# DCGM/pero-pretraining

Hardware: AMD Instinct MI355X
Metric: text-line images/sec (masked-ViT step) (higher is better)
Workload: dtype bf16; 1 GPU; masked pretraining step incl. prepare_batch, 12-layer d=512 h=4 ff=2048 ViT, V=4096, 40x2048 u8 lines (BASELINE.json configs[1]); uint8 images resident in HBM, the PCIe-inclusive rate is `with_h2d`; lines_per_gpu=2048, global_batch=2048, seq_len=256, parallelism=dp1, optimizer=fused Adam (f32 master weights), weight_gradients_on_side_stream=False, head_rows=all, head_backward=masked

## Files before the change

pero_pretraining_amd/csrc/attention.hip:

```cpp
#include "common.hpp"

#define AT_HALF_BYTES 16384
#ifndef AT_NO_PRIO
#define AT_PRIO(n_) __builtin_amdgcn_s_setprio(n_)
#else
#define AT_PRIO(n_)
#endif
#define AT_SUB_BYTES 8192
#ifndef AT_COLSUM_MFMA
#define AT_COLSUM_MFMA 1
#endif
#ifndef AT_ABL
#define AT_ABL 0
#endif
#define AT_DKV2_LDS (4 * AT_SUB_BYTES + 128 * 128 * 2 + 512)
#define AT_TILE_BYTES (128 * 128 * 2)

template <bool VIMG>
__device__ __forceinline__ void attn_glds_tile(const bf16raw* g, long long ld, unsigned char* lds, int wave, int lane) {
#pragma unroll
  for (int i = 0; i < 8; i++) {
    const int p = wave + 4 * i;
    const int row = 4 * p + (lane >> 4), slot = lane & 15;
    const int chunk = VIMG ? ((((slot >> 2) ^ (row & 3)) << 2) | (slot & 3)) : (slot ^ (row & 15));
// ... 1418 lines not shown
  bf8v qf[8];
  const unsigned qoff = (unsigned)((long long)q * ld * 2 + 16 * h5);
  auto load_q = [&](int head) {
    const bf16raw* qb_ = lbase + head * 128;
    at_static_for<0, 8>([&](auto kc) __attribute__((always_inline)) { constexpr int ks = decltype(kc)::value; lh_gload16<32 * ks>(qf[ks], qb_, qoff); });
  };
  load_q(head0);
  const unsigned kbase = at_lds_addr(kimg), vbase = at_lds_addr(vimg);
  const unsigned ka0 = (unsigned)(r * 256 + ((h5 ^ (r & 15)) << 4));
  unsigned va0;
  {
    const int i = lane & 15, g1 = (lane >> 4) & 1;
    const int key = 4 * h5 + (i >> 2);
    va0 = (unsigned)(key * 256 + ((key & 3) << 6) + g1 * 32 + (i & 3) * 8);
  }
  f16v o[4];
#pragma unroll
  for (int t = 0; t < 4; t++) o[t] = (f16v){0};
  float m = -INFINITY, l = 0.f;

  for (int u = 0; u < units; u++) {
    const int head = head0 + u / nkt, kt = u % nkt;
    if (u > 0) asm volatile("s_waitcnt vmcnt(8)" ::: "memory");
    else asm volatile("s_waitcnt vmcnt(0)" ::: "memory");
    asm volatile("" : "+v"(qf[0]), "+v"(qf[1]), "+v"(qf[2]), "+v"(qf[3]), "+v"(qf[4]), "+v"(qf[5]), "+v"(qf[6]), "+v"(qf[7]) :: "memory");
    lh_barrier();
    bf8v fr[FW_POOL];
    f16v s[4];
    auto issue_k = [&](auto jc) __attribute__((always_inline)) {
      constexpr int j = decltype(jc)::value;
      constexpr int t = j >> 3, ks = j & 7;
      at_rd128x<t * 8192, 32 * ks>(fr[j % FW_POOL], ka0, kbase);
    };
    at_static_for<0, 6>(issue_k);
    AT_PRIO(1);
    at_static_for<0, 32>([&](auto jc) __attribute__((always_inline)) {
      constexpr int j = decltype(jc)::value;
      constexpr int t = j >> 3, ks = j & 7;
      if constexpr (j + 6 < 32) issue_k(std::integral_constant<int, j + 6>{});
      constexpr int after = (31 - j) < 6 ? (31 - j) : 6;
      at_wait_lgkm<after>(fr[j % FW_POOL]);
      if constexpr (ks == 0) s[t] = __builtin_amdgcn_mfma_f32_32x32x16_bf16(fr[j % FW_POOL], qf[0], (f16v){0}, 0, 0, 0);
      else s[t] = __builtin_amdgcn_mfma_f32_32x32x16_bf16(fr[j % FW_POOL], qf[ks], s[t], 0, 0, 0);
    });
    AT_PRIO(0);
    asm volatile("s_waitcnt vmcnt(0)" ::: "memory");
    lh_barrier();
    if (u + 1 < units) {
      const int nhd = head0 + (u + 1) / nkt, nkt_i = (u + 1) % nkt;
      attn_glds_tile<false>(lbase + nhd * 128 + d + (long long)nkt_i * 128 * ld, ld, kimg, wave, lane);
    }
    auto issue_v = [&](auto mc) __attribute__((always_inline)) {
      constexpr int mm = decltype(mc)::value;
      constexpr int t = mm >> 3, sub = (mm >> 2) & 1, dt = mm & 3;
      at_rdtrx<t * 8192 + sub * 4096, t * 8192 + sub * 4096 + 2048, 64 * dt>(fr[mm % FW_POOL], va0, va0, vbase);
    };
    at_static_for<0, 7>(issue_v);

    float mx = s[0][0];
#pragma unroll
    for (int t = 0; t < 4; t++)
#pragma unroll
      for (int e = 0; e < 16; e++) mx = fmaxf(mx, s[t][e]);
    {
      const auto sw = __builtin_amdgcn_permlane32_swap(__float_as_uint(mx), __float_as_uint(mx), false, false);
      mx = fmaxf(__uint_as_float(sw[0]), __uint_as_float(sw[1]));
    }
    const float mn = fmaxf(m, mx);
    const float alpha = __builtin_amdgcn_exp2f((m - mn) * c);
    const float mc = mn * c;
    float ps = 0.f;
#pragma unroll
    for (int t = 0; t < 4; t++)
#pragma unroll
      for (int e = 0; e < 16; e++) {
        const float p = __builtin_amdgcn_exp2f(fmaf(s[t][e], c, -mc));
        s[t][e] = p;
        ps += p;
      }
    {
      const auto sw = __builtin_amdgcn_permlane32_swap(__float_as_uint(ps), __float_as_uint(ps), false, false);
      ps = __uint_as_float(sw[0]) + __uint_as_float(sw[1]);
    }
    l = l * alpha + ps;
    m = mn;
    if (kt != 0) {
#pragma unroll
      for (int t = 0; t < 4; t++)
#pragma unroll
        for (int e = 0; e < 16; e++) o[t][e] *= alpha;
    }

    AT_PRIO(1);
    at_static_for<0, 32>([&](auto mc_) __attribute__((always_inline)) {
      constexpr int mm = decltype(mc_)::value;
      constexpr int t = mm >> 3, sub = (mm >> 2) & 1, dt = mm & 3;
      if constexpr (mm + 7 < 32) issue_v(std::integral_constant<int, mm + 7>{});
      constexpr int after = 2 * ((31 - mm) < 7 ? (31 - mm) : 7);
      at_wait_lgkm<after>(fr[mm % FW_POOL]);
      const bf8v pf = pack8(s[t], sub);
      o[dt] = __builtin_amdgcn_mfma_f32_32x32x16_bf16(fr[mm % FW_POOL], pf, o[dt], 0, 0, 0);
    });
    AT_PRIO(0);
    if (kt == nkt - 1) {
      lh_barrier();
      const float inv = 1.0f / l;
      int qrow_l = wave * 32 + r, tid_l = tid;
      asm volatile("" : "+v"(qrow_l), "+v"(tid_l));
#pragma unroll
      for (int dt = 0; dt < 4; dt++)
#pragma unroll
        for (int g4 = 0; g4 < 4; g4++) {
          const at_u2v w = {pack2bf(o[dt][4 * g4 + 0] * inv, o[dt][4 * g4 + 1] * inv), pack2bf(o[dt][4 * g4 + 2] * inv, o[dt][4 * g4 + 3] * inv)};
          const int g = dt * 8 + 2 * g4 + h5;
          lh_ds_write8(vbase + qrow_l * 256 + ((g ^ (qrow_l & 31)) << 3), w);
        }
      lh_gstore4(m * c + __builtin_amdgcn_logf(l), lse2 + ((long long)line * nh + head) * S, (unsigned)q * 4u);
      lh_wait_lgkm_plain<0>();
      lh_barrier();
      {
        const int ch = tid_l & 15;
        at_u4v v[8];
#pragma unroll
        for (int i = 0; i < 8; i++) {
          const int row = (tid_l >> 4) + 16 * i;
          lh_ds_read16(v[i], vbase + row * 256 + ((ch ^ ((row & 31) >> 1)) << 4));
        }
        asm volatile("s_waitcnt lgkmcnt(0)" : "+v"(v[0]), "+v"(v[1]), "+v"(v[2]), "+v"(v[3]), "+v"(v[4]), "+v"(v[5]), "+v"(v[6]), "+v"(v[7]) :: "memory");
#pragma unroll
        for (int i = 0; i < 8; i++) {
          const int row = (tid_l >> 4) + 16 * i;
          at_u4v x = v[i];
          if (row & 1) x = (at_u4v){v[i][2], v[i][3], v[i][0], v[i][1]};
          lh_gstore16<0>(x, out + ((long long)line * S + qb * 128) * d + head * 128, (unsigned)(row * (int)d * 2 + ch * 16));
        }
      }
      if (u + 1 < units) {
#pragma unroll
        for (int t = 0; t < 4; t++) o[t] = (f16v){0};
        m = -INFINITY;
        l = 0.f;
        load_q(head + 1);
      }
    }
    if (u + 1 < units) {
      lh_barrier();
      const int nhd = head0 + (u + 1) / nkt, nkt_i = (u + 1) % nkt;
      attn_glds_tile<true>(lbase + nhd * 128 + 2 * d + (long long)nkt_i * 128 * ld, ld, vimg, wave, lane);
    }
  }
}


int g_attn_bwd_pair = 1;
int g_attn_order = 32;
int g_attn_lh = 0;
int g_attn_pipe = 1;
extern "C" int pero_attention_bwd(const void* qkv, const void* out, const void* dout, const float* lse, float* dvec, void* dqkv,
                                  float* dbias, float* work, int64_t N, int64_t S, int64_t num_heads, int64_t head_dim, int dtype,
                                  void* stream) {
  PERO_REQUIRE(qkv && dout && lse && dvec && dqkv, "pero_attention_bwd: null pointer");
  PERO_REQUIRE(dtype == PERO_BF16 && head_dim == 128 && S % 128 == 0 && S > 0 && N > 0 && num_heads > 0,
               "pero_attention_bwd: fused kernel needs bf16, head_dim 128, S %% 128 == 0");
  PERO_REQUIRE(aligned16(qkv) && (!out || aligned16(out)) && aligned16(dout) && aligned16(dqkv), "pero_attention_bwd: 16-byte alignment");
  PERO_REQUIRE(!dbias || work, "pero_attention_bwd: dbias needs the partial-sum workspace");
  PERO_LDS_ATTR(attn_bwd_dq_k<false>, 2 * AT_TILE_BYTES);
  PERO_LDS_ATTR(attn_bwd_dq_k<true>, 2 * AT_TILE_BYTES);
  PERO_LDS_ATTR(attn_bwd_dkv2_k<false>, AT_DKV2_LDS);
  PERO_LDS_ATTR(attn_bwd_dkv2_k<true>, AT_DKV2_LDS);
  PERO_LDS_ATTR(attn_bwd_pair_k<false>, AT_DKV2_LDS > 2 * AT_TILE_BYTES ? AT_DKV2_LDS : 2 * AT_TILE_BYTES);
  PERO_LDS_ATTR(attn_bwd_pair_k<true>, AT_DKV2_LDS > 2 * AT_TILE_BYTES ? AT_DKV2_LDS : 2 * AT_TILE_BYTES);
  const float scale = (float)(1.0 / sqrt((double)head_dim));
  const float c = (float)(1.4426950408889634 / sqrt((double)head_dim));
  hipStream_t st = (hipStream_t)stream;
  dim3 grid((unsigned)(N * num_heads * (S / 128))), block(256);
  if (!out && g_attn_bwd_pair && g_attn_lh && S == 256 && dbias && N * num_heads < (1LL << 20) && num_heads <= 1024) {
#ifdef LH_STAMP
#define LH_LAUNCH_LDS (LH_LDS_BYTES + 512)
#else
#define LH_LAUNCH_LDS LH_LDS_BYTES
#endif
    PERO_LDS_ATTR(attn_bwd_lh_k, LH_LAUNCH_LDS);
    const long long units = N * num_heads;
    const int cus = pero_num_cus();
    hipLaunchKernelGGL(attn_bwd_lh_k, dim3((unsigned)(units < cus ? units : cus)), dim3(512), LH_LAUNCH_LDS, st, (const bf16raw*)qkv, (const bf16raw*)dout, lse,
                       (const float*)dvec, (bf16raw*)dqkv, work, (int)units, (int)num_heads, c, scale);
    hipLaunchKernelGGL(attn_bias_reduce_k, dim3((unsigned)num_heads, 3, N >= 4096 ? 128 : N >= 1024 ? 64 : 16), dim3(128), 0, st, work, dbias, (int)N, (int)num_heads, 1);
    PERO_CHECK_LAUNCH("pero_attention_bwd");
    return PERO_OK;
  }
  if (!out && g_attn_bwd_pair) {
    const size_t lds = AT_DKV2_LDS > 2 * AT_TILE_BYTES ? AT_DKV2_LDS : 2 * AT_TILE_BYTES;
    if (g_attn_pipe)
      hipLaunchKernelGGL(attn_bwd_pair_k<true>, dim3(2 * grid.x), block, lds, st, (const bf16raw*)qkv, (const bf16raw*)dout, lse, dvec, (bf16raw*)dqkv,
                         dbias ? work : nullptr, (int)S, (int)num_heads, c, scale, g_attn_order);
    else
      hipLaunchKernelGGL(attn_bwd_pair_k<false>, dim3(2 * grid.x), block, lds, st, (const bf16raw*)qkv, (const bf16raw*)dout, lse, dvec, (bf16raw*)dqkv,
                         dbias ? work : nullptr, (int)S, (int)num_heads, c, scale, g_attn_order);
  } else {
  if (g_attn_pipe)
    hipLaunchKernelGGL(attn_bwd_dq_k<true>, grid, block, 2 * AT_TILE_BYTES, st, (const bf16raw*)qkv, (const bf16raw*)out, (const bf16raw*)dout, lse,
                       dvec, (bf16raw*)dqkv, dbias ? work : nullptr, (int)S, (int)num_heads, c, scale);
  else
    hipLaunchKernelGGL(attn_bwd_dq_k<false>, grid, block, 2 * AT_TILE_BYTES, st, (const bf16raw*)qkv, (const bf16raw*)out, (const bf16raw*)dout, lse,
                       dvec, (bf16raw*)dqkv, dbias ? work : nullptr, (int)S, (int)num_heads, c, scale);
  if (g_attn_pipe)
    hipLaunchKernelGGL(attn_bwd_dkv2_k<true>, grid, block, AT_DKV2_LDS, st, (const bf16raw*)qkv, (const bf16raw*)dout, lse, dvec,
                       (bf16raw*)dqkv, dbias ? work : nullptr, (int)S, (int)num_heads, c, scale);
  else
    hipLaunchKernelGGL(attn_bwd_dkv2_k<false>, grid, block, AT_DKV2_LDS, st, (const bf16raw*)qkv, (const bf16raw*)dout, lse, dvec,
                       (bf16raw*)dqkv, dbias ? work : nullptr, (int)S, (int)num_heads, c, scale);
  }
  if (dbias)
    hipLaunchKernelGGL(attn_bias_reduce_k, dim3((unsigned)num_heads, 3, (N * (S / 128) >= 4096) ? 128 : (N * (S / 128) >= 1024) ? 64 : 16), dim3(128), 0, st, work, dbias, (int)N, (int)num_heads, (int)(S / 128));
  PERO_CHECK_LAUNCH("pero_attention_bwd");
  return PERO_OK;
}
```

pero_pretraining_amd/csrc/gemm.hip:

```cpp
#include "common.hpp"

#include "gemm_common.hpp"
#include <string.h>

#define T_BM 128
#define T_BN 128
#define T_BK 64
#define T_OPBYTES (128 * 64 * 2)
#define T_BUFBYTES (2 * T_OPBYTES)
#define T_EPI_PITCH 528
#define T_LDS_BYTES (128 * T_EPI_PITCH)

__device__ __forceinline__ bf8v frag_rowmajor(const unsigned char* base, int row, int ks, int lane) {
  const int r = row + (lane & 15);
  const int chunk = ks * 4 + (lane >> 4);
  return *(const bf8v*)(base + r * 128 + ((chunk ^ (r & 7)) << 4));
}
__device__ __forceinline__ bf8v frag_kmajor(const unsigned char* base, int col, int ks, int lane) {
  const int i = lane & 15;
  const int krow = ks * 32 + 8 * (lane >> 4) + (i >> 2);
  const unsigned char* a = base + krow * 256 + ((((col >> 4) ^ fk(krow))) << 5) + 8 * (i & 3);
  s4v lo = __builtin_amdgcn_ds_read_tr16_b64_v4i16(LDS_PTR(s4v, a));
  s4v hi = __builtin_amdgcn_ds_read_tr16_b64_v4i16(LDS_PTR(s4v, a + 4 * 256));
  typedef short s8v __attribute__((ext_vector_type(8)));
// ... 135 lines not shown
          case 5: STORE_PREV_BATCH(5); break;
          case 6: STORE_PREV_BATCH(6); break;
          case 7: STORE_PREV_BATCH(7); break;
          default: break;
        }
      }
      const unsigned char* sa = smem + buf * T_BUFBYTES;
      const unsigned char* sb = sa + T_OPBYTES;
      unsigned char* da = smem + (buf ^ 1) * T_BUFBYTES;
      if (t + 1 < it.nk) {
        stage_glds<TA>(it.A, p.lda, it.tm0, it.kbeg + (long long)(t + 1) * T_BK, da, tid);
        stage_glds<TB>(it.B, p.ldb, it.tn0, it.kbeg + (long long)(t + 1) * T_BK, da + T_OPBYTES, tid);
      } else if (have_next && !atomic) {
        stage_glds<TA>(nx.A, p.lda, nx.tm0, nx.kbeg, da, tid);
        stage_glds<TB>(nx.B, p.ldb, nx.tn0, nx.kbeg, da + T_OPBYTES, tid);
      }
#pragma unroll
      for (int ks = 0; ks < 2; ks++) {
        bf8v fa[4], fb[4];
#pragma unroll
        for (int i = 0; i < 4; i++) {
          fa[i] = TA ? frag_kmajor(sa, wm * 64 + i * 16, ks, lane) : frag_rowmajor(sa, wm * 64 + i * 16, ks, lane);
          fb[i] = TB ? frag_kmajor(sb, wn * 64 + i * 16, ks, lane) : frag_rowmajor(sb, wn * 64 + i * 16, ks, lane);
        }
#pragma unroll
        for (int i = 0; i < 4; i++)
#pragma unroll
          for (int j = 0; j < 4; j++)
            acc[i][j] = __builtin_amdgcn_mfma_f32_16x16x32_bf16(fb[j], fa[i], acc[i][j], 0, 0, 0);
      }
      buf ^= 1;
    }
    if (have_prev && it.nk < 8) {
      if (it.nk <= 0) STORE_PREV_BATCH(0);
      if (it.nk <= 1) STORE_PREV_BATCH(1);
      if (it.nk <= 2) STORE_PREV_BATCH(2);
      if (it.nk <= 3) STORE_PREV_BATCH(3);
      if (it.nk <= 4) STORE_PREV_BATCH(4);
      if (it.nk <= 5) STORE_PREV_BATCH(5);
      if (it.nk <= 6) STORE_PREV_BATCH(6);
      if (it.nk <= 7) STORE_PREV_BATCH(7);
    }
    have_prev = false;

    if (atomic) {
      lds_barrier();
#pragma unroll
      for (int i = 0; i < 4; i++)
#pragma unroll
        for (int j = 0; j < 4; j++)
          *(f4v*)(smem + (lm + i * 16) * T_EPI_PITCH + (ln + j * 16) * 4) = acc[i][j];
      lds_barrier();
      float* C = (float*)p.C + it.coff;
#pragma unroll 4
      for (int i = 0; i < 32; i++) {
        const int row = wave + 4 * i;
#pragma unroll
        for (int j = 0; j < 2; j++) {
          const int col = lane + 64 * j;
          const float v = *(const float*)(smem + row * T_EPI_PITCH + col * 4) * p.alpha;
          atomicAdd(C + (it.tm0 + row) * p.ldc + it.tn0 + col, v);
        }
      }
      if (have_next) {
        lds_barrier();
        stage_glds<TA>(nx.A, p.lda, nx.tm0, nx.kbeg, smem, tid);
        stage_glds<TB>(nx.B, p.ldb, nx.tn0, nx.kbeg, smem + T_OPBYTES, tid);
        buf = 0;
      }
    } else {
#pragma unroll
      for (int i = 0; i < 4; i++)
#pragma unroll
        for (int j = 0; j < 4; j++) prev[i][j] = acc[i][j];
      pm = it.tm0 + lm; pn = it.tn0 + ln; pcoff = it.coff;
      have_prev = true;
    }
    if (!have_next) break;
    w = wnext;
    it = nx;
  }
  if (have_prev) {
#pragma unroll
    for (int b = 0; b < 8; b++) { STORE_PREV_BATCH(b); }
  }
#undef STORE_PREV
#undef STORE_PREV_BATCH
}

template <typename TI, typename TO>
__global__ __launch_bounds__(256) void gemm_generic(GemmP p) {
  __shared__ float As[64][17];
  __shared__ float Bs[64][17];
  const int tid = threadIdx.x, lane = tid & 63, wave = tid >> 6;
  const int wm = wave >> 1, wn = wave & 1;
  const long long tm0 = (long long)blockIdx.x * 64, tn0 = (long long)blockIdx.y * 64;
  const int b = blockIdx.z;
  const long long bo = b / p.binner, bi = b % p.binner;
  const TI* A = (const TI*)p.A + bo * p.sAo + bi * p.sAi;
  const TI* B = (const TI*)p.B + bo * p.sBo + bi * p.sBi;
  const long long coff = bo * p.sCo + bi * p.sCi;
  const bool ta = p.flags & PERO_GEMM_TRANS_A, tb = p.flags & PERO_GEMM_TRANS_B;
  const long long sam = ta ? 1 : p.lda, sak = ta ? p.lda : 1;
  const long long sbn = tb ? 1 : p.ldb, sbk = tb ? p.ldb : 1;

  f16v acc = {0};
  for (long long k0 = 0; k0 < p.K; k0 += 16) {
#pragma unroll
    for (int i = 0; i < 4; i++) {
      const int idx = tid + 256 * i;
      int m, k;
      if (ta) { m = idx & 63; k = idx >> 6; } else { m = idx >> 4; k = idx & 15; }
      float v = 0.f;
      if (tm0 + m < p.M && k0 + k < p.K) v = Elem<TI>::ld(A + (tm0 + m) * sam + (k0 + k) * sak);
      As[m][k] = v;
      int n, k2;
      if (tb) { n = idx & 63; k2 = idx >> 6; } else { n = idx >> 4; k2 = idx & 15; }
      float w = 0.f;
      if (tn0 + n < p.N && k0 + k2 < p.K) w = Elem<TI>::ld(B + (tn0 + n) * sbn + (k0 + k2) * sbk);
      Bs[n][k2] = w;
    }
    __syncthreads();
#pragma unroll
    for (int k = 0; k < 16; k += 2) {
      const float a = As[wm * 32 + (lane & 31)][k + (lane >> 5)];
      const float bb = Bs[wn * 32 + (lane & 31)][k + (lane >> 5)];
      acc = __builtin_amdgcn_mfma_f32_32x32x2f32(a, bb, acc, 0, 0, 0);
    }
    __syncthreads();
  }
  const long long n = tn0 + wn * 32 + (lane & 31);
  if (n >= p.N) return;
  const float bias = p.bias ? p.bias[n] : 0.f;
#pragma unroll
  for (int r = 0; r < 16; r++) {
    const long long m = tm0 + wm * 32 + (r & 3) + 8 * (r >> 2) + 4 * (lane >> 5);
    if (m >= p.M) continue;
    float v = acc[r] * p.alpha + bias;
    if (p.resid) v += Elem<TI>::ld((const TI*)p.resid + coff + m * p.ldr + n);
    if (p.flags & PERO_GEMM_RELU) v = fmaxf(v, 0.f);
    if (p.gate && !(Elem<TI>::ld((const TI*)p.gate + coff + m * p.ldg + n) > 0.f)) v = 0.f;
    TO* c = (TO*)p.C + coff + m * p.ldc + n;
    if (sizeof(TO) == 4 && (p.flags & PERO_GEMM_ATOMIC)) atomicAdd((float*)c, v);
    else if (sizeof(TO) == 4 && (p.flags & PERO_GEMM_ACCUM)) *(float*)c += v;
    else Elem<TO>::st(c, v);
  }
}

extern int g_gemm_e_var;
extern int g_attn_bwd_pair;
extern int g_attn_pipe;
extern int g_attn_order;
extern int g_attn_lh;
extern int g_gemm_splitk_ws;
extern int g_gemm_splitk_table;
extern int g_gemm_nw;
extern int g_gemm_d128;
extern int g_gemm_e_walk;
static int g_gemm_policy = 0;
static int g_gemm_e256_min = 192;
static int g_gemm_e_splitk_min = 4;
static int g_splitk_items = 512;
static int g_splitk_nearest = 0;
int g_pero_splitk_xcd = 1;
extern "C" int pero_set_option(const char* name, int value) {
  if (name && !strcmp(name, "gemm_policy")) { g_gemm_policy = value; return PERO_OK; }
  if (name && !strcmp(name, "gemm_e_var")) { g_gemm_e_var = value; return PERO_OK; }
  if (name && !strcmp(name, "attn_bwd_pair")) { g_attn_bwd_pair = value; return PERO_OK; }
  if (name && !strcmp(name, "attn_pipe")) { g_attn_pipe = value; return PERO_OK; }
  if (name && !strcmp(name, "attn_order")) { g_attn_order = value; return PERO_OK; }
  if (name && !strcmp(name, "attn_lh")) { g_attn_lh = value; return PERO_OK; }
  if (name && !strcmp(name, "splitk_workspace")) { g_gemm_splitk_ws = value; return PERO_OK; }
  if (name && !strcmp(name, "splitk_table")) { g_gemm_splitk_table = value; return PERO_OK; }
  if (name && !strcmp(name, "gemm_nw")) { g_gemm_nw = value; return PERO_OK; }
  if (name && !strcmp(name, "gemm_d128")) { g_gemm_d128 = value; return PERO_OK; }
  if (name && !strcmp(name, "gemm_e_walk")) { g_gemm_e_walk = value; return PERO_OK; }
  if (name && !strcmp(name, "gemm_e256_min")) { g_gemm_e256_min = value; return PERO_OK; }
  if (name && !strcmp(name, "gemm_e_splitk_min")) { g_gemm_e_splitk_min = value; return PERO_OK; }
  if (name && !strcmp(name, "splitk_xcd")) { g_pero_splitk_xcd = value; return PERO_OK; }
  if (name && !strcmp(name, "splitk_nearest")) { g_splitk_nearest = value; return PERO_OK; }
  if (name && !strcmp(name, "splitk_items")) { g_splitk_items = value > 0 ? value : 512; return PERO_OK; }
  pero_set_error("pero_set_option: unknown option %s", name ? name : "(null)");
  return PERO_E_INVALID;
}

static int gemm_dispatch(const void* A, const void* B, void* C, const float* bias, const void* residual, const void* gate,
                         int64_t M, int64_t N, int64_t K, int64_t lda, int64_t ldb, int64_t ldc, int64_t ldr, int64_t ldg,
                         int64_t batch, int64_t batch_inner,
                         int64_t sAo, int64_t sAi, int64_t sBo, int64_t sBi, int64_t sCo, int64_t sCi,
                         float alpha, int flags, int k_split, int in_dtype, int out_dtype, void* workspace, int64_t workspace_bytes,
                         void* stream, bool* colsum_fused);

static bool splitk_takes_e256(int64_t M, int64_t N, int64_t K, int flags) {
  const bool can256 = M % 256 == 0 && N % 256 == 0 && !(flags & PERO_GEMM_TILE128) && g_gemm_policy != 1;
  const long long t256 = can256 ? (M / 256) * (N / 256) : 0;
  return can256 && K % 64 == 0 && K >= 128 &&
         (g_gemm_policy == 20 || (g_gemm_policy == 0 && ((flags & PERO_GEMM_TILE256) || (g_gemm_e256_min > 0 && K >= 32768 && t256 >= g_gemm_e_splitk_min))));
}
extern "C" int pero_gemm_resid_layernorm(const void* A, const void* W, const float* bias, const void* R, const float* gamma, const float* beta,
                                         void* Y, void* T, float* mean, float* rstd, int64_t M, int64_t N, int64_t K, int64_t lda, int64_t ldw,
                                         int64_t ldy, int64_t ldr, int64_t ldt, float eps, void* stream) {
  PERO_REQUIRE(A && W && R && gamma && beta && T && mean && rstd, "pero_gemm_resid_layernorm: null pointer");
  PERO_REQUIRE(N == 512 && M > 0 && M % 128 == 0 && K % 64 == 0 && K >= 192 && lda % 8 == 0 && ldw % 8 == 0 && (!Y || ldy % 8 == 0) && ldr % 8 == 0 &&
               ldt % 8 == 0 && aligned16(A) && aligned16(W) && aligned16(R) && (!Y || aligned16(Y)) && aligned16(T) && aligned16(gamma) && aligned16(beta) &&
               (!bias || aligned16(bias)),
               "pero_gemm_resid_layernorm: bf16, N = 512, M %% 128 == 0, K %% 64 == 0, K >= 192, 16-byte aligned rows");
  GemmP p;
  p.A = A; p.B = W; p.C = Y; p.bias = bias; p.resid = R; p.gate = nullptr;
  p.M = M; p.N = N; p.K = K; p.lda = lda; p.ldb = ldw; p.ldc = Y ? ldy : 512; p.ldr = ldr; p.ldg = 0;
  p.sAo = p.sAi = p.sBo = p.sBi = p.sCo = p.sCi = 0;
  p.binner = 1; p.alpha = 1.0f; p.flags = 0; p.kchunk = K;
  PERO_REQUIRE(pero_launch_gemm_n512_ln(p, T, ldt, mean, rstd, gamma, beta, eps, (hipStream_t)stream), "pero_gemm_resid_layernorm: shape not taken");
  PERO_CHECK_LAUNCH("pero_gemm_resid_layernorm");
  return PERO_OK;
}
extern "C" int pero_gemm_resid_layernorm_bwd(const void* A, const void* Wt, const void* R, const void* T, const float* rstd, const float* gamma,
                                             const float* beta, void* DX, float* dgamma, float* dbeta, float* dxsum, float* work, int64_t M, int64_t N,
                                             int64_t K, int64_t lda, int64_t ldw, int64_t ldr, int64_t ldt, int64_t lddx, void* stream) {
  PERO_REQUIRE(A && Wt && R && T && rstd && gamma && beta && DX && dgamma && dbeta && work, "pero_gemm_resid_layernorm_bwd: null pointer");
  PERO_REQUIRE(N == 512 && M > 0 && M % 128 == 0 && K % 64 == 0 && K >= 192 && lda % 8 == 0 && ldw % 8 == 0 && ldr % 8 == 0 && ldt % 8 == 0 &&
               lddx % 8 == 0 && aligned16(A) && aligned16(Wt) && aligned16(R) && aligned16(T) && aligned16(DX) && aligned16(gamma) && aligned16(beta),
               "pero_gemm_resid_layernorm_bwd: bf16, N = 512, M %% 128 == 0, K %% 64 == 0, K >= 192, 16-byte aligned rows");
  GemmP p;
  p.A = A; p.B = Wt; p.C = DX; p.bias = nullptr; p.resid = R; p.gate = nullptr;
  p.M = M; p.N = N; p.K = K; p.lda = lda; p.ldb = ldw; p.ldc = lddx; p.ldr = ldr; p.ldg = 0;
  p.sAo = p.sAi = p.sBo = p.sBi = p.sCo = p.sCi = 0;
  p.binner = 1; p.alpha = 1.0f; p.flags = 0; p.kchunk = K;
  int grid = 0;
  PERO_REQUIRE(pero_launch_gemm_n512_lnb(p, T, ldt, rstd, gamma, beta, work, &grid, (hipStream_t)stream), "pero_gemm_resid_layernorm_bwd: shape not taken");
  pero_ln_bwd_reduce_launch(work, dgamma, dbeta, dxsum, grid, 512, (hipStream_t)stream);
  PERO_CHECK_LAUNCH("pero_gemm_resid_layernorm_bwd");
  return PERO_OK;
}
extern "C" int64_t pero_gemm_workspace_bytes(int64_t M, int64_t N, int64_t K, int64_t batch, int flags, int k_split, int in_dtype,
                                             int out_dtype) {
  if (!(flags & PERO_GEMM_ATOMIC) || batch != 1 || in_dtype != PERO_BF16 || out_dtype != PERO_F32 || (flags & PERO_GEMM_FORCE_GENERIC) || M <= 0 ||
      N <= 0 || K <= 0 || !splitk_takes_e256(M, N, K, flags))
    return 0;
  return pero_gemm_e256_splitk_ws_bytes(M, N, K, k_split);
}

extern "C" int pero_gemm(const void* A, const void* B, void* C, const float* bias, const void* residual, const void* gate,
                         int64_t M, int64_t N, int64_t K, int64_t lda, int64_t ldb, int64_t ldc, int64_t ldr, int64_t ldg,
                         int64_t batch, int64_t batch_inner,
                         int64_t sAo, int64_t sAi, int64_t sBo, int64_t sBi, int64_t sCo, int64_t sCi,
                         float alpha, int flags, int k_split, int in_dtype, int out_dtype, void* workspace, int64_t workspace_bytes,
                         void* stream) {
  bool fused = false;
  PERO_REQUIRE(workspace_bytes >= 0 && (workspace || workspace_bytes == 0), "pero_gemm: workspace_bytes without a workspace");
  if (flags & PERO_GEMM_COLSUM)
    PERO_REQUIRE(bias && batch == 1 && !(flags & (PERO_GEMM_ATOMIC | PERO_GEMM_ACCUM | PERO_GEMM_ROWDOT)),
                 "pero_gemm: PERO_GEMM_COLSUM needs the output pointer in `bias`, one problem, a stored result");
  if (flags & PERO_GEMM_ROWDOT)
    PERO_REQUIRE(bias && gate && batch == 1 && out_dtype == PERO_BF16 && N % 128 == 0 && !(flags & (PERO_GEMM_ATOMIC | PERO_GEMM_ACCUM)),
                 "pero_gemm: PERO_GEMM_ROWDOT needs the output pointer in `bias`, the second matrix in `gate`, bf16 C, N %% 128 == 0");
  const int rc = gemm_dispatch(A, B, C, bias, residual, gate, M, N, K, lda, ldb, ldc, ldr, ldg, batch, batch_inner, sAo, sAi, sBo, sBi,
                               sCo, sCi, alpha, flags, k_split, in_dtype, out_dtype, workspace, workspace_bytes, stream, &fused);
  if (rc != PERO_OK || !(flags & (PERO_GEMM_COLSUM | PERO_GEMM_ROWDOT)) || fused) return rc;
  if (flags & PERO_GEMM_ROWDOT) return pero_rowdot_blocks(C, gate, (float*)bias, M, N, ldc, ldg, stream);
  return pero_colsum(C, (float*)bias, M, N, ldc, out_dtype, stream);
}

static int gemm_dispatch(const void* A, const void* B, void* C, const float* bias, const void* residual, const void* gate,
                         int64_t M, int64_t N, int64_t K, int64_t lda, int64_t ldb, int64_t ldc, int64_t ldr, int64_t ldg,
                         int64_t batch, int64_t batch_inner,
                         int64_t sAo, int64_t sAi, int64_t sBo, int64_t sBi, int64_t sCo, int64_t sCi,
                         float alpha, int flags, int k_split, int in_dtype, int out_dtype, void* workspace, int64_t workspace_bytes,
                         void* stream, bool* colsum_fused) {
  PERO_REQUIRE(A && B && C, "pero_gemm: null operand");
  PERO_REQUIRE(M > 0 && N > 0 && K > 0 && batch > 0 && batch_inner > 0, "pero_gemm: bad sizes M=%lld N=%lld K=%lld batch=%lld",
               (long long)M, (long long)N, (long long)K, (long long)batch);
  PERO_REQUIRE((in_dtype == PERO_F32 || in_dtype == PERO_BF16) && (out_dtype == PERO_F32 || out_dtype == PERO_BF16), "pero_gemm: bad dtype");
  PERO_REQUIRE(!((flags & (PERO_GEMM_ATOMIC | PERO_GEMM_ACCUM)) && out_dtype != PERO_F32), "pero_gemm: ATOMIC/ACCUM need f32 C");
  PERO_REQUIRE(k_split >= 0 && (k_split == 1 || (flags & PERO_GEMM_ATOMIC)), "pero_gemm: k_split != 1 needs PERO_GEMM_ATOMIC");
  PERO_REQUIRE(batch < 65536, "pero_gemm: batch too large");
  const bool ta = flags & PERO_GEMM_TRANS_A, tb = flags & PERO_GEMM_TRANS_B;
  GemmP p;
  p.A = A; p.B = B; p.C = C; p.bias = bias; p.resid = residual; p.gate = gate;
  p.M = M; p.N = N; p.K = K; p.lda = lda; p.ldb = ldb; p.ldc = ldc; p.ldr = ldr; p.ldg = ldg;
  p.sAo = sAo; p.sAi = sAi; p.sBo = sBo; p.sBi = sBi; p.sCo = sCo; p.sCi = sCi;
  p.binner = (int)batch_inner; p.alpha = alpha; p.flags = flags; p.kchunk = K;
  hipStream_t st = (hipStream_t)stream;
  const bool want_cs = flags & (PERO_GEMM_COLSUM | PERO_GEMM_ROWDOT);
  const bool want_rd = flags & PERO_GEMM_ROWDOT;
  const int cs_bits = flags & (PERO_GEMM_COLSUM | PERO_GEMM_ROWDOT);
  GemmP pc = p;
  if (want_cs) { flags &= ~(PERO_GEMM_COLSUM | PERO_GEMM_ROWDOT); p.flags = flags; p.bias = nullptr; if (want_rd) p.gate = nullptr; }

  const int esz_o = out_dtype == PERO_F32 ? 4 : 2;
  bool fast = in_dtype == PERO_BF16 && !(flags & 32) && M % T_BM == 0 && N % T_BN == 0 && K % T_BK == 0 &&
              lda % 8 == 0 && ldb % 8 == 0 && (ldc * esz_o) % 16 == 0 && aligned16(A) && aligned16(B) && aligned16(C) &&
              (sAo % 8 == 0) && (sAi % 8 == 0) && (sBo % 8 == 0) && (sBi % 8 == 0) && ((sCo * esz_o) % 16 == 0) &&
              ((sCi * esz_o) % 16 == 0) && (!residual || (ldr % 8 == 0 && aligned16(residual))) &&
              (!gate || (flags & PERO_GEMM_RELU_BITS) || (ldg % 8 == 0 && aligned16(gate))) && (!(residual || gate) || out_dtype == PERO_BF16 || true);
  if (fast && g_gemm_policy == 1) { flags |= PERO_GEMM_TILE128; p.flags = flags; pc.flags = flags | cs_bits; }
  const bool force128 = flags & PERO_GEMM_TILE128, force256 = flags & PERO_GEMM_TILE256;
  PERO_REQUIRE(!(flags & PERO_GEMM_MASK_TILED) || ((flags & PERO_GEMM_RELU_BITS) && N % 256 == 0), "pero_gemm: PERO_GEMM_MASK_TILED needs PERO_GEMM_RELU_BITS and N %% 256 == 0");
  if (flags & PERO_GEMM_RELU_BITS) {
    PERO_REQUIRE(fast && gate && batch == 1 && out_dtype == PERO_BF16 && !ta && !(flags & PERO_GEMM_ATOMIC) && !force128 && M % 256 == 0 &&
                 N % 128 == 0 && K % 32 == 0 && !(flags & PERO_GEMM_ROWDOT) && (g_gemm_policy == 0 || g_gemm_policy == 7 || g_gemm_policy == 20),
                 "pero_gemm: PERO_GEMM_RELU_BITS needs a bf16 product for the 256-row tile kernels (M %% 256, N %% 128, K %% 32, batch 1)");
  }
  if (fast) {
    const bool atomic = flags & PERO_GEMM_ATOMIC;
    const bool can256 = M % 256 == 0 && N % 256 == 0 && !force128;
    const long long t256 = can256 ? (M / 256) * (N / 256) * batch : 0;
    const long long t128 = (M / T_BM) * (N / T_BN) * batch;
    const int k_split_req = k_split;
    const bool auto_or = g_gemm_policy == 0;
    if (atomic && out_dtype == PERO_F32 && batch == 1 && splitk_takes_e256(M, N, K, flags) &&
        pero_launch_gemm_e256(p, batch, k_split_req, ta, tb, true, st, -1, workspace, workspace_bytes)) {
      PERO_CHECK_LAUNCH("pero_gemm(e256 split-K)");
      return PERO_OK;
    }
    if (!atomic && g_gemm_nw && !want_cs && out_dtype == PERO_BF16 && pero_launch_gemm_n512(p, batch, ta, tb, false, st)) {
      PERO_CHECK_LAUNCH("pero_gemm(n512)");
      return PERO_OK;
    }
    if (!atomic && g_gemm_d128 && out_dtype == PERO_BF16 && !want_rd && K <= g_gemm_d128 * 64LL && (auto_or || g_gemm_policy == 20) &&
        pero_launch_gemm_d128(pc, batch, ta, tb, false, st)) {
      *colsum_fused = want_cs;
      PERO_CHECK_LAUNCH("pero_gemm(d128)");
      return PERO_OK;
    }
// ... 69 lines not shown
```

Measured before the change: 14190 lines/s.

## Add one-pass fused attention backward kernel for S=256, enabled by default

Adds a new attention-backward kernel that computes dQ, dK, dV and the bias-gradient partials in a single pass per (line, head). K stays resident in LDS, while Q/dO stages and the LSE/dvec statistics are double-buffered. dQ is accumulated through a dS strip in LDS and handled by alternating wave groups. It replaces the two-block pair kernel for S=256, which is meant to remove the repeated loads of Q/K/V/dO and the separate dQ pass. In exchange it uses about 145KB of LDS and 512-thread blocks, which may limit occupancy.

```diff
diff --git a/pero_pretraining_amd/csrc/attention.hip b/pero_pretraining_amd/csrc/attention.hip
--- a/pero_pretraining_amd/csrc/attention.hip
+++ b/pero_pretraining_amd/csrc/attention.hip
@@ -1594,10 +1594,254 @@
 }
 
 
+#define OP_K 0
+#define OP_ST 65536
+#define OP_STAT (OP_ST + 2 * 16384)
+#define OP_STRIP (OP_STAT + 512)
+#define OP_DQS (OP_STRIP + 2 * 16384)
+#define OP_LDS_BYTES (OP_DQS + 2 * 8192)
+#ifndef OP_RDEPTH
+#define OP_RDEPTH 4
+#endif
+#ifndef OP_TDEPTH
+#define OP_TDEPTH 4
+#endif
+
+__device__ __forceinline__ void op_glds(const bf16raw* g, long long ld, unsigned char* lds, int npieces, int wave, int lane) {
+  asm volatile("" : "+v"(lane));
+  for (int p = wave; p < npieces; p += 8) {
+    const int row = 4 * p + (lane >> 4), slot = lane & 15;
+    const int chunk = slot ^ img_f(row);
+    __builtin_amdgcn_global_load_lds((const __attribute__((address_space(1))) void*)((const unsigned char*)g + (unsigned)(row * (int)ld * 2 + chunk * 16)),
+                                     (__attribute__((address_space(3))) void*)(lds + p * 1024), 16, 0, 0);
+  }
+}
+
+__global__ __launch_bounds__(512, 2) void attn_bwd_1p_k(const bf16raw* qkv, const bf16raw* dout, const float* lse2, const float* dvec,
+                                                        bf16raw* dqkv, float* dbias, int nh, float c, float scale) {
+  extern __shared__ __attribute__((aligned(16))) unsigned char smem[];
+  constexpr int S = 256, NST = 8;
+  const int tid = threadIdx.x, lane = tid & 63, h5 = lane >> 5, r = lane & 31;
+  const int wave = __builtin_amdgcn_readfirstlane(tid >> 6), grp = wave >> 2, wi = wave & 3;
+  const int lh = blockIdx.x, line = lh / nh, head = lh % nh;
+  const long long d = (long long)nh * 128, ld = 3 * d;
+  const long long nwg = (long long)gridDim.x * 2;
+  const bf16raw* base = qkv + (long long)line * S * ld + head * 128;
+  const bf16raw* Gg = dout + (long long)line * S * d + head * 128;
+  const int key = 32 * wave + r;
+  const unsigned s0 = at_lds_addr(smem);
+
+  op_glds(base + d, ld, smem + OP_K, 64, wave, lane);
+  auto issue_stage = [&](int j) {
+    unsigned char* st = smem + OP_ST + (j & 1) * 16384;
+    if (wave == 0) {
+      const float* sp = lane < 32 ? lse2 + (long long)lh * S + j * 32 + lane : dvec + ((long long)line * S + j * 32 + (lane & 31)) * nh + head;
+      __builtin_amdgcn_global_load_lds((const __attribute__((address_space(1))) void*)sp,
+                                       (__attribute__((address_space(3))) void*)(smem + OP_STAT + (j & 1) * 256), 4, 0, 0);
+    }
+    op_glds(base + (long long)j * 32 * ld, ld, st, 8, wave, lane);
+    op_glds(Gg + (long long)j * 32 * d, d, st + 8192, 8, wave, lane);
+  };
+  issue_stage(0);
+  bf8v vf[8];
+  {
+    const bf16raw* vrow = base + 2 * d + (long long)key * ld + 8 * h5;
+#pragma unroll
+    for (int ks = 0; ks < 8; ks++) vf[ks] = *(const bf8v*)(vrow + 16 * ks);
+  }
+
+  const unsigned ra0 = (unsigned)(r * 256 + ((h5 ^ img_f(r)) << 4));
+  unsigned ta0, tb0, sa0, sb0;
+  {
+    const int i = lane & 15, g1 = (lane >> 4) & 1;
+    const int row = 4 * h5 + (i >> 2);
+    const int ch = 2 * g1 + ((i & 3) >> 1);
+    ta0 = (unsigned)(row * 256 + ((ch ^ img_f(row)) << 4) + 8 * (i & 1));
+    tb0 = (unsigned)((row + 8) * 256 + ((ch ^ img_f(row + 8)) << 4) + 8 * (i & 1));
+    sa0 = (unsigned)(row * 64 + ((ch ^ h5) << 4) + 8 * (i & 1));
+    sb0 = (unsigned)((row + 8) * 64 + ((ch ^ h5 ^ 2) << 4) + 8 * (i & 1));
+  }
+  const unsigned tad = ta0 ^ (64u * wi), tbd = tb0 ^ (64u * wi);
+  const unsigned kbase = s0 + OP_K + wave * 8192;
+  const unsigned strip_w = (unsigned)(key * 64 + 8 * h5), strip_x = (unsigned)((key >> 2) & 3);
+  const __bf16 one = (__bf16)1.0f;
+  const bf8v ones = {one, one, one, one, one, one, one, one};
+  float colacc = 0.f;
+
+  f16v dv[4], dk[4];
+#pragma unroll
+  for (int t = 0; t < 4; t++) { dv[t] = (f16v){0}; dk[t] = (f16v){0}; }
+
+  auto store_dq = [&](int j) {
+    const unsigned stg = s0 + OP_DQS + (j & 1) * 8192;
+    int tq = tid;
+    asm volatile("" : "+v"(tq));
+    const int row = tq >> 4, ch = tq & 15;
+    at_u4v v;
+    lh_ds_read16(v, stg + row * 256 + ((ch ^ (row >> 1)) << 4));
+    bf8v fa, fb;
+    if (wave < 4 && dbias) {
+      const int ti = lane & 15, tg = (lane >> 4) & 1;
+      const int g = 8 * wave + 4 * tg + (ti & 3);
+      const int q0 = 8 * h5 + (ti >> 2);
+      const int r0 = q0, r1 = q0 + 4, r2 = 16 + q0, r3 = 20 + q0;
+      at_rdtra<0, 0>(fa, stg + r0 * 256 + ((g ^ r0) << 3), stg + r1 * 256 + ((g ^ r1) << 3));
+      at_rdtra<0, 0>(fb, stg + r2 * 256 + ((g ^ r2) << 3), stg + r3 * 256 + ((g ^ r3) << 3));
+    }
+    asm volatile("s_waitcnt lgkmcnt(0)" : "+v"(v), "+v"(fa), "+v"(fb) :: "memory");
+    if (row & 1) v = (at_u4v){v[2], v[3], v[0], v[1]};
+    *(at_u4v*)((unsigned char*)(dqkv + ((long long)line * S + j * 32) * ld + head * 128) + (unsigned)(row * (int)ld * 2 + ch * 16)) = v;
+    if (wave < 4 && dbias) {
+      f16v cs = __builtin_amdgcn_mfma_f32_32x32x16_bf16(ones, fa, (f16v){0}, 0, 0, 0);
+      cs = __builtin_amdgcn_mfma_f32_32x32x16_bf16(ones, fb, cs, 0, 0, 0);
+      colacc += cs[0];
+      if ((j & 3) == 3) {
+        int ln = lane;
+        asm volatile("" : "+v"(ln));
+        if (ln < 32) dbias[((long long)lh * 2 + (j >> 2)) * 128 + 32 * wave + ln] = colacc;
+        colacc = 0.f;
+      }
+    }
+  };
+
+  for (int it = 0; it <= NST; it++) {
+    asm volatile("s_waitcnt vmcnt(0) lgkmcnt(0)" ::: "memory");
+    asm volatile("" : "+v"(vf[0]), "+v"(vf[1]), "+v"(vf[2]), "+v"(vf[3]), "+v"(vf[4]), "+v"(vf[5]), "+v"(vf[6]), "+v"(vf[7]) :: "memory");
+    lh_barrier();
+    if (it >= 2) store_dq(it - 2);
+    if (it + 1 < NST) issue_stage(it + 1);
+
+    if (it >= 1 && grp == ((it - 1) & 1)) {
+      const unsigned strip = s0 + OP_STRIP + ((it - 1) & 1) * 16384;
+      const unsigned kimg = s0 + OP_K;
+      bf8v fr[OP_TDEPTH + 2];
+      f16v dq;
+      auto issue_q = [&](auto jc) __attribute__((always_inline)) {
+        constexpr int j = decltype(jc)::value;
+        constexpr int kb = 16 * (j >> 1);
+        if constexpr ((j & 1) == 0) at_rdtr<kb * 256, kb * 256>(fr[j % (OP_TDEPTH + 2)], tad, tbd, kimg);
+        else at_rdtr<kb * 64, kb * 64>(fr[j % (OP_TDEPTH + 2)], sa0, sb0, strip);
+      };
+      at_static_for<0, OP_TDEPTH>(issue_q);
+      AT_PRIO(1);
+      at_static_for<0, 32>([&](auto jc) __attribute__((always_inline)) {
+        constexpr int j = decltype(jc)::value;
+        if constexpr (j + OP_TDEPTH < 32) issue_q(std::integral_constant<int, j + OP_TDEPTH>{});
+        if constexpr (j & 1) {
+          constexpr int after = 2 * ((31 - j) < OP_TDEPTH ? (31 - j) : OP_TDEPTH);
+          at_wait_lgkm<after>(fr[j % (OP_TDEPTH + 2)]);
+          asm volatile("" : "+v"(fr[(j - 1) % (OP_TDEPTH + 2)]));
+          if constexpr (j == 1) dq = __builtin_amdgcn_mfma_f32_32x32x16_bf16(fr[0], fr[1], (f16v){0}, 0, 0, 0);
+          else dq = __builtin_amdgcn_mfma_f32_32x32x16_bf16(fr[(j - 1) % (OP_TDEPTH + 2)], fr[j % (OP_TDEPTH + 2)], dq, 0, 0, 0);
+        }
+      });
+      AT_PRIO(0);
+      const unsigned stg = s0 + OP_DQS + ((it - 1) & 1) * 8192 + r * 256;
+#pragma unroll
+      for (int g4 = 0; g4 < 4; g4++) {
+        const at_u2v w = {pack2bf(dq[4 * g4 + 0], dq[4 * g4 + 1]), pack2bf(dq[4 * g4 + 2], dq[4 * g4 + 3])};
+        lh_ds_write8(stg + (((wi * 8 + 2 * g4 + h5) ^ r) << 3), w);
+      }
+    }
+    if (it == NST) break;
+
+    const unsigned stage = s0 + OP_ST + (it & 1) * 16384;
+    f16v s, dp;
+    {
+      constexpr int P = OP_RDEPTH + 2;
+      bf8v fr[P];
+      auto issue_r = [&](auto jc) __attribute__((always_inline)) {
+        constexpr int j = decltype(jc)::value;
+        constexpr int ks = j / 3, kind = j % 3;
+        if constexpr (kind == 0) at_rd128x<0, 32 * ks>(fr[j % P], ra0, stage);
+        else if constexpr (kind == 1) at_rd128x<0, 32 * ks>(fr[j % P], ra0, kbase);
+        else at_rd128x<8192, 32 * ks>(fr[j % P], ra0, stage);
+      };
+      at_static_for<0, OP_RDEPTH>(issue_r);
+      AT_PRIO(1);
+      at_static_for<0, 24>([&](auto jc) __attribute__((always_inline)) {
+        constexpr int j = decltype(jc)::value;
+        constexpr int ks = j / 3, kind = j % 3;
+        if constexpr (j + OP_RDEPTH < 24) issue_r(std::integral_constant<int, j + OP_RDEPTH>{});
+        constexpr int after = (23 - j) < OP_RDEPTH ? (23 - j) : OP_RDEPTH;
+        if constexpr (kind == 1) {
+          at_wait_lgkm<after>(fr[j % P]);
+          asm volatile("" : "+v"(fr[(j - 1) % P]));
+          if constexpr (ks == 0) s = __builtin_amdgcn_mfma_f32_32x32x16_bf16(fr[(j - 1) % P], fr[j % P], (f16v){0}, 0, 0, 0);
+          else s = __builtin_amdgcn_mfma_f32_32x32x16_bf16(fr[(j - 1) % P], fr[j % P], s, 0, 0, 0);
+        } else if constexpr (kind == 2) {
+          at_wait_lgkm<after>(fr[j % P]);
+          if constexpr (ks == 0) dp = __builtin_amdgcn_mfma_f32_32x32x16_bf16(fr[j % P], vf[0], (f16v){0}, 0, 0, 0);
+          else dp = __builtin_amdgcn_mfma_f32_32x32x16_bf16(fr[j % P], vf[ks], dp, 0, 0, 0);
+        }
+      });
+      AT_PRIO(0);
+    }
+    bf8v pf[2], dsf[2];
+    {
+      const unsigned stb = s0 + OP_STAT + (it & 1) * 256, sto = 16 * h5;
+      at_static_for<0, 4>([&](auto gc) __attribute__((always_inline)) {
+        constexpr int g4 = decltype(gc)::value;
+        f4v l4, d4;
+        at_rd128<32 * g4>(l4, sto, stb);
+        at_rd128<128 + 32 * g4>(d4, sto, stb);
+        at_wait_lgkm2<0>(l4, d4);
+#pragma unroll
+        for (int e = 0; e < 4; e++) {
+          const float p = __builtin_amdgcn_exp2f(fmaf(s[4 * g4 + e], c, -l4[e]));
+          s[4 * g4 + e] = p;
+          dp[4 * g4 + e] = p * (dp[4 * g4 + e] - d4[e]) * scale;
+        }
+      });
+      pf[0] = pack8(s, 0); dsf[0] = pack8(dp, 0);
+      pf[1] = pack8(s, 1); dsf[1] = pack8(dp, 1);
+    }
+    {
+      const unsigned strip = s0 + OP_STRIP + (it & 1) * 16384 + strip_w;
+#pragma unroll
+      for (int g = 0; g < 4; g++) {
+        const at_u4v u = __builtin_bit_cast(at_u4v, dsf[g >> 1]);
+        const at_u2v w = {u[2 * (g & 1)], u[2 * (g & 1) + 1]};
+        lh_ds_write8(strip + ((g ^ strip_x) << 4), w);
+      }
+    }
+    {
+      constexpr int P = OP_TDEPTH + 1;
+      bf8v fr[P];
+      auto issue_t = [&](auto mc) __attribute__((always_inline)) {
+        constexpr int m = decltype(mc)::value;
+        constexpr int sub = m >> 3, dt = (m >> 1) & 3, kind = m & 1;
+        constexpr int off = sub * 4096 + (kind == 0 ? 8192 : 0);
+        at_rdtrx<off, off, 64 * dt>(fr[m % P], ta0, tb0, stage);
+      };
+      at_static_for<0, OP_TDEPTH>(issue_t);
+      AT_PRIO(1);
+      at_static_for<0, 16>([&](auto mc) __attribute__((always_inline)) {
+        constexpr int m = decltype(mc)::value;
+        constexpr int sub = m >> 3, dt = (m >> 1) & 3, kind = m & 1;
+        if constexpr (m + OP_TDEPTH < 16) issue_t(std::integral_constant<int, m + OP_TDEPTH>{});
+        constexpr int after = 2 * ((15 - m) < OP_TDEPTH ? (15 - m) : OP_TDEPTH);
+        at_wait_lgkm<after>(fr[m % P]);
+        if constexpr (kind == 0) dv[dt] = __builtin_amdgcn_mfma_f32_32x32x16_bf16(fr[m % P], pf[sub], dv[dt], 0, 0, 0);
+        else dk[dt] = __builtin_amdgcn_mfma_f32_32x32x16_bf16(fr[m % P], dsf[sub], dk[dt], 0, 0, 0);
+      });
+      AT_PRIO(0);
+    }
+  }
+  asm volatile("s_waitcnt lgkmcnt(0)" ::: "memory");
+  lh_barrier();
+  store_dq(NST - 1);
+  bf16raw* tile_o = dqkv + ((long long)line * S + grp * 128) * ld + d + head * 128;
+  unsigned char* stg = smem + OP_K + grp * 32768;
+  attn_store_tile(dk, stg, tile_o, ld, dbias ? dbias + (nwg + (long long)lh * 2 + grp) * 128 : nullptr, tid & 255, wi, r, h5);
+  attn_store_tile(dv, stg, tile_o + d, ld, dbias ? dbias + (2 * nwg + (long long)lh * 2 + grp) * 128 : nullptr, tid & 255, wi, r, h5);
+}
+
 int g_attn_bwd_pair = 1;
 int g_attn_order = 32;
 int g_attn_lh = 0;
 int g_attn_pipe = 1;
+int g_attn_onepass = 1;
 extern "C" int pero_attention_bwd(const void* qkv, const void* out, const void* dout, const float* lse, float* dvec, void* dqkv,
                                   float* dbias, float* work, int64_t N, int64_t S, int64_t num_heads, int64_t head_dim, int dtype,
                                   void* stream) {
@@ -1631,7 +1875,11 @@
     PERO_CHECK_LAUNCH("pero_attention_bwd");
     return PERO_OK;
   }
-  if (!out && g_attn_bwd_pair) {
+  if (!out && g_attn_bwd_pair && g_attn_onepass && S == 256 && N * num_heads < (1LL << 20) && num_heads <= 1024) {
+    PERO_LDS_ATTR(attn_bwd_1p_k, OP_LDS_BYTES);
+    hipLaunchKernelGGL(attn_bwd_1p_k, dim3((unsigned)(N * num_heads)), dim3(512), OP_LDS_BYTES, st, (const bf16raw*)qkv, (const bf16raw*)dout, lse,
+                       (const float*)dvec, (bf16raw*)dqkv, dbias ? work : nullptr, (int)num_heads, c, scale);
+  } else if (!out && g_attn_bwd_pair) {
     const size_t lds = AT_DKV2_LDS > 2 * AT_TILE_BYTES ? AT_DKV2_LDS : 2 * AT_TILE_BYTES;
     if (g_attn_pipe)
       hipLaunchKernelGGL(attn_bwd_pair_k<true>, dim3(2 * grid.x), block, lds, st, (const bf16raw*)qkv, (const bf16raw*)dout, lse, dvec, (bf16raw*)dqkv,
diff --git a/pero_pretraining_amd/csrc/gemm.hip b/pero_pretraining_amd/csrc/gemm.hip
--- a/pero_pretraining_amd/csrc/gemm.hip
+++ b/pero_pretraining_amd/csrc/gemm.hip
@@ -311,6 +311,7 @@
 extern int g_attn_pipe;
 extern int g_attn_order;
 extern int g_attn_lh;
+extern int g_attn_onepass;
 extern int g_gemm_splitk_ws;
 extern int g_gemm_splitk_table;
 extern int g_gemm_nw;
@@ -329,6 +330,7 @@
   if (name && !strcmp(name, "attn_pipe")) { g_attn_pipe = value; return PERO_OK; }
   if (name && !strcmp(name, "attn_order")) { g_attn_order = value; return PERO_OK; }
   if (name && !strcmp(name, "attn_lh")) { g_attn_lh = value; return PERO_OK; }
+  if (name && !strcmp(name, "attn_onepass")) { g_attn_onepass = value; return PERO_OK; }
   if (name && !strcmp(name, "splitk_workspace")) { g_gemm_splitk_ws = value; return PERO_OK; }
   if (name && !strcmp(name, "splitk_table")) { g_gemm_splitk_table = value; return PERO_OK; }
   if (name && !strcmp(name, "gemm_nw")) { g_gemm_nw = value; return PERO_OK; }
```

Measured after the change: 14420 lines/s (median of 6 runs). 1.6% higher.
